# NoemieJaquier/GaBOtorch

Measured on AMD Instinct MI355X. Metric: SPD affine-invariant kernel-matrix build, pairs/sec (N=4096,d=10), higher is better.
Workload: dtype f64

## Files before the change

gabotorch_amd/csrc/spd_backward.hip:

```cpp
#include "gabo_device.hpp"
#include "spd_prep.hpp"
#include "spd_eigvec.hpp"
#include "spd_generic.hpp"
#include "../../include/gabo_hip.h"

#ifndef GABO_BWD_TWO_WAVE_MAX_DIM
#define GABO_BWD_TWO_WAVE_MAX_DIM 8
#endif

namespace gabo {

template <int D>
__global__ __launch_bounds__(64, (D > GABO_BWD_TWO_WAVE_MAX_DIM ? 1 : 2)) void spd_ai_backward_kernel(const double* __restrict__ Winv, const double* __restrict__ G,
                                                             const double* __restrict__ gout, double* __restrict__ gx,
                                                             int64_t n1, int64_t n2, int64_t w_batch_stride,
                                                             int64_t g_batch_stride, int64_t go_sb, int64_t go_si, int64_t go_sj,
                                                             double beta, int flags) {
    constexpr int T = tri_size(D);
    __shared__ double acc[T * 64];
    __shared__ double red[T];
    __shared__ double wl[T];
    const int mode = flags & GABO_OUT_MASK;
    const int lane = threadIdx.x;
    const int64_t b = blockIdx.x / n1;
    const int64_t i = blockIdx.x - b * n1;
    const double* W = Winv + b * w_batch_stride + i * T;
    static_for<T>([&](auto ee) { acc[decltype(ee)::value * 64 + lane] = 0.0; });
    for (int64_t j0 = 0; j0 < n2; j0 += 64) {
        const int64_t j = j0 + lane;
        const bool live = j < n2;
        const int64_t jc = live ? j : n2 - 1;
        const double* Gj = G + b * g_batch_stride + jc;
        double m[T];
        static_for<T>([&](auto ee) { m[decltype(ee)::value] = 0.0; });
        static_for<D>([&](auto cc) {
            constexpr int col = decltype(cc)::value;
            double g[D - col], c[D - col];
            static_for<D - col>([&](auto kk) { g[decltype(kk)::value] = Gj[(int64_t)tri(col + decltype(kk)::value, col) * n2]; });
            static_for<D - col>([&](auto rr) {
                constexpr int r = col + decltype(rr)::value;
                double a = W[tri(r, col)] * g[0];
                static_for<r - col>([&](auto kk) {
                    constexpr int k = col + 1 + decltype(kk)::value;
                    a = __builtin_fma(W[tri(r, k)], g[k - col], a);
                });
                c[r - col] = a;
            });
            static_for<D - col>([&](auto rr) {
                constexpr int r = col + decltype(rr)::value;
                static_for<r - col + 1>([&](auto qq) {
                    constexpr int q = col + decltype(qq)::value;
                    m[tri(r, q)] = __builtin_fma(c[r - col], c[q - col], m[tri(r, q)]);
                });
            });
        });
        double vreg[D * D];
        double lam[D];
        {
#ifndef GABO_BWD_QL_EPS2
#define GABO_BWD_QL_EPS2 1e-26
#endif
            double qe = GABO_BWD_QL_EPS2;
            asm volatile("" : "+s"(qe));
#ifndef GABO_BWD_TWO_PASS_MIN_DIM
#define GABO_BWD_TWO_PASS_MIN_DIM 4
#endif
            if constexpr (D >= GABO_BWD_TWO_PASS_MIN_DIM) sym_eig_reg_two_pass<D>(m, lam, vreg, qe);
            else sym_eig_reg<D>(m, lam, vreg, qe);
        }
        auto Vat = [&](int r, int c) -> double { return vreg[r * D + c]; };
        double lg[D];
        double s = 0.0;
        {
            const LogRegs logc = LogRegs::load();
            static_for<D>([&](auto kk) {
                constexpr int k = decltype(kk)::value;
                const double l = log_pos(lam[k], logc);
                lg[k] = lam[k] > 0.0 ? l : __builtin_nan("");
                s = __builtin_fma(lg[k], lg[k], s);
            });
        }
        double d2 = s + 1e-15;
        double go = live ? gout[b * go_sb + i * go_si + j * go_sj] : 0.0;
        double w;
        if (mode == GABO_OUT_GAUSSIAN) {
            double dist = __builtin_sqrt(d2);
            w = go * (-beta) * exp(-((dist * dist) * beta));
        } else if (mode == GABO_OUT_LAPLACE) {
            double dist = __builtin_sqrt(d2);
            w = go * (-beta) * exp(-(dist * beta)) / (2.0 * dist);
        } else {
            w = go / (2.0 * __builtin_sqrt(d2));
        }
        static_for<D>([&](auto rr) {
            constexpr int r = decltype(rr)::value;
            double vl[D];
            static_for<D>([&](auto kk) { vl[decltype(kk)::value] = Vat(r, decltype(kk)::value) * (w * lg[decltype(kk)::value]); });
            static_for<r + 1>([&](auto cc) {
                constexpr int c = decltype(cc)::value;
                double f = acc[tri(r, c) * 64 + lane];
                static_for<D>([&](auto kk) { constexpr int k = decltype(kk)::value; f = __builtin_fma(vl[k], Vat(c, k), f); });
                acc[tri(r, c) * 64 + lane] = f;
            });
        });
    }
    __syncthreads();
    for (int e = lane; e < T; e += 64) {
        double t = 0.0;
        for (int l = 0; l < 64; ++l) t += acc[e * 64 + ((l + e) & 63)];
        red[e] = t;
    }
    for (int e = lane; e < T; e += 64) wl[e] = W[e];
    __syncthreads();
    for (int e = lane; e < T; e += 64) {
        int a = 0;
        while (tri(a + 1, 0) <= e) ++a;
        int bb = e - tri(a, 0);
        double t = 0.0;
        for (int r = a; r < D; ++r) {
            double inner = 0.0;
            for (int c = bb; c < D; ++c) {
                double srs = r >= c ? red[tri(r, c)] : red[tri(c, r)];
                inner = __builtin_fma(srs, wl[tri(c, bb)], inner);
            }
            t = __builtin_fma(wl[tri(r, a)], inner, t);
        }
        t *= -2.0;
        gx[(b * n1 + i) * T + mandel_pos(D, a, bb)] = (a == bb) ? t : t * kSqrt2;
    }
}

template <int D>
static int launch_spd_ai_backward(const double* x1, const double* x2, const double* gout, double* gx, int64_t batch, int64_t n1,
                                  int64_t n2, int64_t s1, int64_t s2, int64_t go_sb, int64_t go_si, int64_t go_sj, double beta,
                                  int flags, double* ws, int* status, hipStream_t st) {
    constexpr int T = tri_size(D);
    const int64_t b1 = (s1 == 0) ? 1 : batch;
    const int64_t b2 = (s2 == 0) ? 1 : batch;
    double* W = ws;
    double* G = ws + b1 * n1 * T;
    launch_spd_prep<D>(x1, x2, W, G, b1, b2, n1, n2, s1, s2, status, st);
    int64_t nblocks = batch * n1;
    if (nblocks > 0x7fffffffLL) return GABO_ERR_ARG;
    hipLaunchKernelGGL((spd_ai_backward_kernel<D>), dim3((unsigned)nblocks), dim3(64), 0, st, W, G, gout, gx, n1, n2,
                       (s1 == 0) ? (int64_t)0 : n1 * T, (s2 == 0) ? (int64_t)0 : n2 * T, go_sb, go_si, go_sj, beta, flags);
    return hipGetLastError() == hipSuccess ? GABO_OK : GABO_ERR_LAUNCH;
}

int launch_spd_ai_backward_duo(int d, const double* x1, const double* x2, const double* gout, double* gx, int64_t batch, int64_t n1, int64_t n2,
                               int64_t s1, int64_t s2, int64_t go_sb, int64_t go_si, int64_t go_sj, double beta, int flags, double* ws, int* status,
                               hipStream_t st);

}

#ifndef GABO_BWD_DUO_MIN_DIM
#define GABO_BWD_DUO_MIN_DIM 12
#endif

extern "C" int gabo_spd_ai_backward(const double* x1, const double* x2, const double* grad_out, double* grad_x1, int64_t batch,
                                    int64_t n1, int64_t n2, int d, int64_t x1_batch_stride, int64_t x2_batch_stride,
                                    int64_t go_batch_stride, int64_t go_row_stride, int64_t go_col_stride, double beta, int flags,
                                    void* workspace, size_t workspace_bytes, int* status, gabo_stream_t stream) {
    if (batch < 0 || n1 < 0 || n2 < 0 || x1_batch_stride < 0 || x2_batch_stride < 0) return GABO_ERR_ARG;
    if (d < 2 || d > GABO_SPD_MAX_DIM) return GABO_ERR_DIM;
    if (batch == 0 || n1 == 0) return GABO_OK;
    if (!x1 || !grad_x1 || !workspace || !status) return GABO_ERR_ARG;
    if (n2 > 0 && (!x2 || !grad_out)) return GABO_ERR_ARG;
    if (workspace_bytes < gabo_spd_ai_workspace_bytes(batch, n1, n2, d)) return GABO_ERR_ARG;
    if (flags & GABO_SYMMETRIC) return GABO_ERR_ARG;
    hipStream_t st = (hipStream_t)stream;
    double* ws = (double*)workspace;
#ifndef GABO_ONLY_DIM
    if (d >= GABO_BWD_DUO_MIN_DIM && d <= GABO_SPD_BWD_REG_MAX_DIM)
        return gabo::launch_spd_ai_backward_duo(d, x1, x2, grad_out, grad_x1, batch, n1, n2, x1_batch_stride, x2_batch_stride, go_batch_stride,
                                                go_row_stride, go_col_stride, beta, flags, ws, status, st);
#endif
    if (d > GABO_SPD_REG_MAX_DIM)
        return gabo::launch_spd_ai_backward_generic(x1, x2, grad_out, grad_x1, batch, n1, n2, d, x1_batch_stride, x2_batch_stride,
                                                    go_batch_stride, go_row_stride, go_col_stride, beta, flags, ws, status, st);
#define GABO_CASE(DD) \
    case DD:          \
        return gabo::launch_spd_ai_backward<DD>(x1, x2, grad_out, grad_x1, batch, n1, n2, x1_batch_stride, x2_batch_stride, \
                                                go_batch_stride, go_row_stride, go_col_stride, beta, flags, ws, status, st);
    switch (d) {
#ifdef GABO_ONLY_DIM
        GABO_CASE(GABO_ONLY_DIM)
#else
        GABO_CASE(2) GABO_CASE(3) GABO_CASE(4) GABO_CASE(5) GABO_CASE(6) GABO_CASE(7) GABO_CASE(8) GABO_CASE(9) GABO_CASE(10)
        GABO_CASE(11) GABO_CASE(12)
#endif
    }
#undef GABO_CASE
    return GABO_ERR_DIM;
}
```

gabotorch_amd/csrc/spd_eigvec.hpp:

```cpp
#pragma once
#include "gabo_device.hpp"

namespace gabo {

template <int D>
__device__ __forceinline__ void tridiagonalize_reflectors(double (&m)[tri_size(D)], double (&dg)[D], double (&e)[D],
                                                          double (&ihh)[D >= 3 ? D - 2 : 1]) {
    static_for<D - 2>([&](auto kk) {
        constexpr int k = decltype(kk)::value;
        constexpr int n = D - k - 1;
        double alpha = m[tri(k + 1, k)];
        double sig = 0.0;
        static_for<n - 1>([&](auto t) { double x = m[tri(k + 2 + decltype(t)::value, k)]; sig = __builtin_fma(x, x, sig); });
        double nn = __builtin_fma(alpha, alpha, sig);
        double nrm = sqrt_pos(nn);
        double u[n];
        u[0] = alpha + copysign_d(nrm, alpha);
        static_for<n - 1>([&](auto t) { u[decltype(t)::value + 1] = m[tri(k + 2 + decltype(t)::value, k)]; });
        double hh = __builtin_fma(__builtin_fabs(alpha), nrm, nn);
        double inv_hh = hh == 0.0 ? 0.0 : rcp(hh);
        double p[n];
        static_for<n>([&](auto rr) {
            constexpr int r = decltype(rr)::value;
            double acc = 0.0;
            static_for<n>([&](auto cc) {
                constexpr int c = decltype(cc)::value;
                constexpr int hi = r > c ? r : c, lo = r > c ? c : r;
                acc = __builtin_fma(m[tri(k + 1 + hi, k + 1 + lo)], u[c], acc);
            });
            p[r] = acc * inv_hh;
        });
        double up = 0.0;
        static_for<n>([&](auto rr) { up = __builtin_fma(u[decltype(rr)::value], p[decltype(rr)::value], up); });
        double kap = 0.5 * up * inv_hh;
        static_for<n>([&](auto rr) { p[decltype(rr)::value] = __builtin_fma(-kap, u[decltype(rr)::value], p[decltype(rr)::value]); });
        static_for<n>([&](auto rr) {
            constexpr int r = decltype(rr)::value;
            static_for<r + 1>([&](auto cc) {
                constexpr int c = decltype(cc)::value;
                double v = m[tri(k + 1 + r, k + 1 + c)];
                v = __builtin_fma(-u[r], p[c], v);
                v = __builtin_fma(-p[r], u[c], v);
                m[tri(k + 1 + r, k + 1 + c)] = v;
            });
        });
        dg[k] = m[tri(k, k)];
        e[k] = hh == 0.0 ? alpha : -copysign_d(nrm, alpha);
        m[tri(k + 1, k)] = u[0];
        ihh[k] = inv_hh;
    });
    if constexpr (D >= 2) {
        dg[D - 2] = m[tri(D - 2, D - 2)];
        e[D - 2] = m[tri(D - 1, D - 2)];
    }
    dg[D - 1] = m[tri(D - 1, D - 1)];
    e[D - 1] = 0.0;
}

template <int D>
__device__ __forceinline__ void tridiagonalize_q(double (&m)[tri_size(D)], double (&dg)[D], double (&e)[D], double (&z)[D * D]) {
    double ihh[D >= 3 ? D - 2 : 1];
    tridiagonalize_reflectors<D>(m, dg, e, ihh);
    static_for<D>([&](auto rr) {
        static_for<D>([&](auto cc) { z[decltype(rr)::value * D + decltype(cc)::value] = (decltype(rr)::value == decltype(cc)::value) ? 1.0 : 0.0; });
    });
    static_for_down<D - 3, 0>([&](auto kk) {
        constexpr int k = decltype(kk)::value;
        constexpr int n = D - k - 1;
        static_for<n>([&](auto cc) {
            constexpr int c = k + 1 + decltype(cc)::value;
            double t = 0.0;
            static_for<n>([&](auto rr) {
                constexpr int r = k + 1 + decltype(rr)::value;
                t = __builtin_fma(m[tri(r, k)], z[r * D + c], t);
            });
            t *= ihh[k];
            static_for<n>([&](auto rr) {
                constexpr int r = k + 1 + decltype(rr)::value;
                z[r * D + c] = __builtin_fma(-m[tri(r, k)], t, z[r * D + c]);
            });
        });
    });
}

template <int D, int ROWS = D, bool VEC = true>
__device__ __forceinline__ void tridiag_ql_vectors(double (&dg)[D], double (&e)[D], double (&z)[ROWS * D], const double eps2_arg = 0.0) {
    const double eps2 = eps2_arg > 0.0 ? eps2_arg : 1.2e-32;
    static_for<D - 1>([&](auto ll) {
        constexpr int l = decltype(ll)::value;
        for (int it = 0; it < 60; ++it) {
            const double s01 = __builtin_fabs(dg[l]) + __builtin_fabs(dg[l + 1]);
            const bool done0 = e[l] * e[l] <= eps2 * (s01 * s01);
            if (__builtin_amdgcn_ballot_w64(done0) == __builtin_amdgcn_ballot_w64(true)) break;
            const double el = done0 ? 0.0 : e[l];
            double sa = dg[l], sb = dg[l + 1], se = el;
            bool idle = done0;
            if constexpr (l + 1 <= D - 2) {
                const double s12 = __builtin_fabs(dg[l + 1]) + __builtin_fabs(dg[l + 2]);
                const bool done1 = e[l + 1] * e[l + 1] <= eps2 * (s12 * s12);
                idle = done0 && done1;
                sa = done0 ? dg[l + 1] : sa;
                sb = done0 ? dg[l + 2] : sb;
                se = done0 ? e[l + 1] : se;
            }
            if (idle) continue;
            double delta = 0.5 * (sb - sa);
            double root = sqrt_nz(__builtin_fma(delta, delta, se * se));
            double sigma = sa - copysign_d(root - __builtin_fabs(delta), delta);
            double g = dg[D - 1] - sigma;
            double s = 1.0, c = 1.0, p = 0.0;
            static_for_down<D - 2, l>([&](auto ii) {
                constexpr int i = decltype(ii)::value;
                const double ei = (i == l) ? el : e[i];
                double f = s * ei;
                double b = c * ei;
                g = copysign_d(__builtin_fmax(__builtin_fabs(g), 1e-150), g);
                double r2 = __builtin_fma(f, f, g * g);
                double ir = rsqrt_nz(r2);
                e[i + 1] = r2 * ir;
                s = f * ir;
                c = g * ir;
                g = dg[i + 1] - p;
                double r = __builtin_fma(dg[i] - g, s, 2.0 * c * b);
                p = s * r;
                dg[i + 1] = g + p;
                g = __builtin_fma(c, r, -b);
                if constexpr (VEC) {
                    static_for<ROWS>([&](auto kk) {
                        constexpr int k = decltype(kk)::value;
                        double zi = z[k * D + i], zj = z[k * D + i + 1];
                        z[k * D + i + 1] = __builtin_fma(s, zi, c * zj);
                        z[k * D + i] = __builtin_fma(c, zi, -s * zj);
                    });
                }
            });
            dg[l] -= p;
            e[l] = g;
            e[D - 1] = 0.0;
        }
    });
}

template <int D, int ROWS = D>
__device__ __forceinline__ void tridiag_ql_vectors_known(double (&dg)[D], double (&e)[D], double (&z)[ROWS * D], const double (&known)[D],
                                                         const double eps2_arg = 0.0) {
    const double eps2 = eps2_arg > 0.0 ? eps2_arg : 1.2e-32;
    static_for<D - 1>([&](auto ll) {
        constexpr int l = decltype(ll)::value;
        for (int it = 0; it < 60; ++it) {
            const double s01 = __builtin_fabs(dg[l]) + __builtin_fabs(dg[l + 1]);
            const bool done0 = e[l] * e[l] <= eps2 * (s01 * s01);
            if (__builtin_amdgcn_ballot_w64(done0) == __builtin_amdgcn_ballot_w64(true)) break;
            if (done0) continue;
            double sigma;
            if (it == 0) {
                sigma = known[l];
            } else {
                const double sa = dg[l], sb = dg[l + 1], se = e[l];
                const double delta = 0.5 * (sb - sa);
                const double root = sqrt_nz(__builtin_fma(delta, delta, se * se));
                sigma = sa - copysign_d(root - __builtin_fabs(delta), delta);
            }
            double g = dg[D - 1] - sigma;
            double s = 1.0, c = 1.0, p = 0.0;
            static_for_down<D - 2, l>([&](auto ii) {
                constexpr int i = decltype(ii)::value;
                const double ei = e[i];
                double f = s * ei;
                double b = c * ei;
                g = copysign_d(__builtin_fmax(__builtin_fabs(g), 1e-150), g);
                double r2 = __builtin_fma(f, f, g * g);
                double ir = rsqrt_nz(r2);
                e[i + 1] = r2 * ir;
                s = f * ir;
                c = g * ir;
                g = dg[i + 1] - p;
                double r = __builtin_fma(dg[i] - g, s, 2.0 * c * b);
                p = s * r;
                dg[i + 1] = g + p;
                g = __builtin_fma(c, r, -b);
                static_for<ROWS>([&](auto kk) {
                    constexpr int k = decltype(kk)::value;
                    double zi = z[k * D + i], zj = z[k * D + i + 1];
                    z[k * D + i + 1] = __builtin_fma(s, zi, c * zj);
                    z[k * D + i] = __builtin_fma(c, zi, -s * zj);
                });
            });
            dg[l] -= p;
            e[l] = g;
            e[D - 1] = 0.0;
        }
    });
}

template <int D>
__device__ __forceinline__ void sym_eig_reg_two_pass(double (&m)[tri_size(D)], double (&lam)[D], double (&v)[D * D], const double eps2 = 0.0) {
    double sub[D], known[D], e1[D], none[D];
    tridiagonalize_q<D>(m, lam, sub, v);
    static_for<D>([&](auto kk) {
        known[decltype(kk)::value] = lam[decltype(kk)::value];
        e1[decltype(kk)::value] = sub[decltype(kk)::value];
    });
    tridiag_ql_vectors<D, 1, false>(known, e1, none, eps2);
    tridiag_ql_vectors_known<D>(lam, sub, v, known, eps2);
}

template <int D>
__device__ __forceinline__ void sym_eig_reg(double (&m)[tri_size(D)], double (&lam)[D], double (&v)[D * D], const double eps2 = 0.0) {
    double sub[D];
    tridiagonalize_q<D>(m, lam, sub, v);
    tridiag_ql_vectors<D>(lam, sub, v, eps2);
}

template <int D>
__device__ __forceinline__ void sym_eig_reg_values(double (&m)[tri_size(D)], double (&lam)[D]) {
    double sub[D], ihh[D >= 3 ? D - 2 : 1], none[D];
    tridiagonalize_reflectors<D>(m, lam, sub, ihh);
    tridiag_ql_vectors<D, 1, false>(lam, sub, none);
}

template <int D>
struct DuoShape {
    static constexpr int HR = (D + 1) / 2;
};

__device__ __forceinline__ double duo_swap(double v) { return dpp_fetch<0xB1, 0xf>(v); }

template <int D>
__device__ __forceinline__ void tridiagonalize_q_duo(double (&m)[tri_size(D)], double (&dg)[D], double (&e)[D],
                                                     double (&zh)[DuoShape<D>::HR * D], bool h) {
    constexpr int HR = DuoShape<D>::HR;
    double ihh[D >= 3 ? D - 2 : 1];
    tridiagonalize_reflectors<D>(m, dg, e, ihh);
    const double one_odd = h ? 1.0 : 0.0, one_even = h ? 0.0 : 1.0;
    static_for<HR>([&](auto rr) {
        constexpr int lr = decltype(rr)::value;
        static_for<D>([&](auto cc) {
            constexpr int c = decltype(cc)::value;
            zh[lr * D + c] = (c == 2 * lr) ? one_even : ((c == 2 * lr + 1) ? one_odd : 0.0);
        });
    });
    static_for_down<D - 3, 0>([&](auto kk) {
        constexpr int k = decltype(kk)::value;
        constexpr int lr0 = k / 2;
        double um[HR];
        static_for<HR - lr0>([&](auto rr) {
            constexpr int lr = lr0 + decltype(rr)::value;
            constexpr int re = 2 * lr, ro = 2 * lr + 1;
            const double ue = (re >= k + 1 && re < D) ? m[tri(re < D ? re : D - 1, k)] : 0.0;
            const double uo = (ro >= k + 1 && ro < D) ? m[tri(ro < D ? ro : D - 1, k)] : 0.0;
            um[lr] = h ? uo : ue;
        });
        static_for<D - k - 1>([&](auto cc) {
            constexpr int c = k + 1 + decltype(cc)::value;
            double t = 0.0;
            static_for<HR - lr0>([&](auto rr) {
                constexpr int lr = lr0 + decltype(rr)::value;
                t = __builtin_fma(um[lr], zh[lr * D + c], t);
            });
            t = (t + duo_swap(t)) * ihh[k];
            static_for<HR - lr0>([&](auto rr) {
                constexpr int lr = lr0 + decltype(rr)::value;
                zh[lr * D + c] = __builtin_fma(-um[lr], t, zh[lr * D + c]);
            });
        });
    });
}

template <int D>
__device__ __forceinline__ void sym_eig_duo(double (&m)[tri_size(D)], double (&lam)[D], double (&vh)[DuoShape<D>::HR * D], bool h) {
    double sub[D];
    tridiagonalize_q_duo<D>(m, lam, sub, vh, h);
    tridiag_ql_vectors<D, DuoShape<D>::HR>(lam, sub, vh);
}

}
```

Baseline: 8.060 billion.

## Use root-free QL first pass and scalar-constant W loads in SPD backward

Replaces the first eigenvalue-only QL pass in the two-pass eigensolver with a root-free (squared off-diagonal) tridiagonal eigenvalue routine, which avoids square roots, or uses hardware sqrt for d=8/10. The second, vector-accumulating pass now runs in reversed index orientation so it matches the ordering of the shifts the new first pass produces. For d>=8 it also reads the per-row W matrix through a constant address-space pointer so the compiler can emit scalar loads. The reversed orientation and the different shift choice can change how fast the iteration converges and its numerical behaviour.

```diff
diff --git a/gabotorch_amd/csrc/spd_backward.hip b/gabotorch_amd/csrc/spd_backward.hip
--- a/gabotorch_amd/csrc/spd_backward.hip
+++ b/gabotorch_amd/csrc/spd_backward.hip
@@ -8,7 +8,28 @@
 #define GABO_BWD_TWO_WAVE_MAX_DIM 8
 #endif
 
+#ifdef GABO_BWD_PARENT_FORM
+#define GABO_BWD_ROOTFREE_FIRST_PASS 0
+#define GABO_BWD_W_PER_CHUNK 0
+#endif
+#ifndef GABO_BWD_ROOTFREE_FIRST_PASS
+#define GABO_BWD_ROOTFREE_FIRST_PASS 1
+#endif
+#ifndef GABO_BWD_W_PER_CHUNK
+#define GABO_BWD_W_PER_CHUNK 1
+#endif
+
 namespace gabo {
+
+__host__ __device__ constexpr bool spd_bwd_rootfree_first_pass(int d) {
+    return GABO_BWD_ROOTFREE_FIRST_PASS != 0 && d >= 4 && d <= 11;
+}
+__host__ __device__ constexpr int spd_bwd_first_pass_sweepctl(int d) {
+    return (d == 8 || d == 10) ? kQlCtlHwSqrt : kQlCtlPlain;
+}
+__host__ __device__ constexpr bool spd_bwd_w_per_chunk(int d) {
+    return GABO_BWD_W_PER_CHUNK != 0 && d >= 8;
+}
 
 template <int D>
 __global__ __launch_bounds__(64, (D > GABO_BWD_TWO_WAVE_MAX_DIM ? 1 : 2)) void spd_ai_backward_kernel(const double* __restrict__ Winv, const double* __restrict__ G,
@@ -31,6 +52,16 @@
         const bool live = j < n2;
         const int64_t jc = live ? j : n2 - 1;
         const double* Gj = G + b * g_batch_stride + jc;
+        typedef const double __attribute__((address_space(4)))* wrow_ptr;
+        const auto Wc = [&] {
+            if constexpr (spd_bwd_w_per_chunk(D)) {
+                wrow_ptr p = (wrow_ptr)W;
+                asm volatile("" : "+s"(p));
+                return p;
+            } else {
+                return W;
+            }
+        }();
         double m[T];
         static_for<T>([&](auto ee) { m[decltype(ee)::value] = 0.0; });
         static_for<D>([&](auto cc) {
@@ -39,10 +70,10 @@
             static_for<D - col>([&](auto kk) { g[decltype(kk)::value] = Gj[(int64_t)tri(col + decltype(kk)::value, col) * n2]; });
             static_for<D - col>([&](auto rr) {
                 constexpr int r = col + decltype(rr)::value;
-                double a = W[tri(r, col)] * g[0];
+                double a = Wc[tri(r, col)] * g[0];
                 static_for<r - col>([&](auto kk) {
                     constexpr int k = col + 1 + decltype(kk)::value;
-                    a = __builtin_fma(W[tri(r, k)], g[k - col], a);
+                    a = __builtin_fma(Wc[tri(r, k)], g[k - col], a);
                 });
                 c[r - col] = a;
             });
@@ -65,7 +96,8 @@
 #ifndef GABO_BWD_TWO_PASS_MIN_DIM
 #define GABO_BWD_TWO_PASS_MIN_DIM 4
 #endif
-            if constexpr (D >= GABO_BWD_TWO_PASS_MIN_DIM) sym_eig_reg_two_pass<D>(m, lam, vreg, qe);
+            if constexpr (D >= GABO_BWD_TWO_PASS_MIN_DIM && spd_bwd_rootfree_first_pass(D)) sym_eig_reg_two_pass_rootfree<D, spd_bwd_first_pass_sweepctl(D)>(m, lam, vreg, qe);
+            else if constexpr (D >= GABO_BWD_TWO_PASS_MIN_DIM) sym_eig_reg_two_pass<D>(m, lam, vreg, qe);
             else sym_eig_reg<D>(m, lam, vreg, qe);
         }
         auto Vat = [&](int r, int c) -> double { return vreg[r * D + c]; };
diff --git a/gabotorch_amd/csrc/spd_eigvec.hpp b/gabotorch_amd/csrc/spd_eigvec.hpp
--- a/gabotorch_amd/csrc/spd_eigvec.hpp
+++ b/gabotorch_amd/csrc/spd_eigvec.hpp
@@ -1,5 +1,6 @@
 #pragma once
 #include "gabo_device.hpp"
+#include "spd_eig.hpp"
 
 namespace gabo {
 
@@ -141,53 +142,59 @@
     });
 }
 
-template <int D, int ROWS = D>
+template <int D, int ROWS = D, bool REV = false>
 __device__ __forceinline__ void tridiag_ql_vectors_known(double (&dg)[D], double (&e)[D], double (&z)[ROWS * D], const double (&known)[D],
                                                          const double eps2_arg = 0.0) {
     const double eps2 = eps2_arg > 0.0 ? eps2_arg : 1.2e-32;
+    constexpr auto di = [](int i) constexpr { return REV ? D - 1 - i : i; };
+    constexpr auto ei = [](int i) constexpr { return REV ? (i == D - 1 ? D - 1 : D - 2 - i) : i; };
     static_for<D - 1>([&](auto ll) {
         constexpr int l = decltype(ll)::value;
         for (int it = 0; it < 60; ++it) {
-            const double s01 = __builtin_fabs(dg[l]) + __builtin_fabs(dg[l + 1]);
-            const bool done0 = e[l] * e[l] <= eps2 * (s01 * s01);
+            const double s01 = __builtin_fabs(dg[di(l)]) + __builtin_fabs(dg[di(l + 1)]);
+            const bool done0 = e[ei(l)] * e[ei(l)] <= eps2 * (s01 * s01);
             if (__builtin_amdgcn_ballot_w64(done0) == __builtin_amdgcn_ballot_w64(true)) break;
             if (done0) continue;
             double sigma;
             if (it == 0) {
                 sigma = known[l];
+                if constexpr (REV && l == D - 2) {
+                    const double c1 = dg[di(D - 1)];
+                    sigma = __builtin_fabs(c1 - known[D - 2]) >= __builtin_fabs(c1 - known[D - 1]) ? known[D - 2] : known[D - 1];
+                }
             } else {
-                const double sa = dg[l], sb = dg[l + 1], se = e[l];
+                const double sa = dg[di(l)], sb = dg[di(l + 1)], se = e[ei(l)];
                 const double delta = 0.5 * (sb - sa);
                 const double root = sqrt_nz(__builtin_fma(delta, delta, se * se));
                 sigma = sa - copysign_d(root - __builtin_fabs(delta), delta);
             }
-            double g = dg[D - 1] - sigma;
+            double g = dg[di(D - 1)] - sigma;
             double s = 1.0, c = 1.0, p = 0.0;
             static_for_down<D - 2, l>([&](auto ii) {
                 constexpr int i = decltype(ii)::value;
-                const double ei = e[i];
-                double f = s * ei;
-                double b = c * ei;
+                const double eo = e[ei(i)];
+                double f = s * eo;
+                double b = c * eo;
                 g = copysign_d(__builtin_fmax(__builtin_fabs(g), 1e-150), g);
                 double r2 = __builtin_fma(f, f, g * g);
                 double ir = rsqrt_nz(r2);
-                e[i + 1] = r2 * ir;
+                e[ei(i + 1)] = r2 * ir;
                 s = f * ir;
                 c = g * ir;
-                g = dg[i + 1] - p;
-                double r = __builtin_fma(dg[i] - g, s, 2.0 * c * b);
+                g = dg[di(i + 1)] - p;
+                double r = __builtin_fma(dg[di(i)] - g, s, 2.0 * c * b);
                 p = s * r;
-                dg[i + 1] = g + p;
+                dg[di(i + 1)] = g + p;
                 g = __builtin_fma(c, r, -b);
                 static_for<ROWS>([&](auto kk) {
                     constexpr int k = decltype(kk)::value;
-                    double zi = z[k * D + i], zj = z[k * D + i + 1];
-                    z[k * D + i + 1] = __builtin_fma(s, zi, c * zj);
-                    z[k * D + i] = __builtin_fma(c, zi, -s * zj);
+                    double zi = z[k * D + di(i)], zj = z[k * D + di(i + 1)];
+                    z[k * D + di(i + 1)] = __builtin_fma(s, zi, c * zj);
+                    z[k * D + di(i)] = __builtin_fma(c, zi, -s * zj);
                 });
             });
-            dg[l] -= p;
-            e[l] = g;
+            dg[di(l)] -= p;
+            e[ei(l)] = g;
             e[D - 1] = 0.0;
         }
     });
@@ -203,6 +210,17 @@
     });
     tridiag_ql_vectors<D, 1, false>(known, e1, none, eps2);
     tridiag_ql_vectors_known<D>(lam, sub, v, known, eps2);
+}
+
+template <int D, int CTL = kQlCtlPlain>
+__device__ __forceinline__ void sym_eig_reg_two_pass_rootfree(double (&m)[tri_size(D)], double (&lam)[D], double (&v)[D * D], const double eps2 = 0.0) {
+    double sub[D], known[D], e2[D];
+    tridiagonalize_q<D>(m, lam, sub, v);
+    static_for<D>([&](auto kk) { known[decltype(kk)::value] = lam[D - 1 - decltype(kk)::value]; });
+    static_for<D - 1>([&](auto kk) { e2[decltype(kk)::value] = sub[D - 2 - decltype(kk)::value] * sub[D - 2 - decltype(kk)::value]; });
+    e2[D - 1] = 0.0;
+    tridiag_eigenvalues<D, kQlOrientCol0, CTL>(known, e2);
+    tridiag_ql_vectors_known<D, D, true>(lam, sub, v, known, eps2);
 }
 
 template <int D>
```

After: 8.059 billion. No clear change (-0.0%).
